# google/neural-light-transport

Hardware: AMD Instinct MI355X
Metric: rendered Mtexels/s at 1024^2 UV (full Model.call forward: U-Net + UV->camera warp); at N > 1: N collective-free replicas of this forward (weak scaling).  The data-parallel TRAIN step with the RCCL gradient all-reduce (BASELINE config 4) is `train_step`: value = Mtexels/s over all ranks, speedup_vs_o (higher is better)
Workload: dtype f32 via 3xbf16 split, 9 exact products, fp32 accumulate (the LDS-tiled encoder convs: fp32 operands as three bf16 terms on v_mfma_f32_16x16x32_bf16, every term product exact in fp32); f32 storage everywhere, every other launch native f32; 1 GPU; BASELINE config 3: dragon_specular relight+view-synth, depth0 16/depth 256, 4 frames/GPU, 1024^2 UV, k=4 obs maps, 512^2 camera warp; frames_per_gpu=4, uv=1024, k=4, cam=512, conv_algo=auto, plan=fused ends, launch=eager, two HIP streams, distinct_batches_rotated=3, launch_tape_replays=0, parallelism=dp1 (frames sharded, no forward collective), world=1, dist_world_size=1, device=cuda:0

## Files before the change

neural-light-transport_amd/csrc/conv_tile3.hip:

```cpp
#include "nlt_common.h"
#include "pack_common.h"

namespace {

typedef __attribute__((ext_vector_type(8))) __bf16 bf16x8;
typedef unsigned short u16;
typedef unsigned int u32x4 __attribute__((ext_vector_type(4)));

constexpr int TH = 8, TW = 16;
constexpr int QS2 = 272, ODD2 = 132;
constexpr int PL = 160;

template <int MODE> struct T3;
template <> struct T3<NLT_CONV_K2S1> { static constexpr int PAIRS = 2, B_UNITS = 153 * 2, B_SLOTS = 6 * PL; };
template <> struct T3<NLT_CONV_K2S2> { static constexpr int PAIRS = 1, B_UNITS = 256 * 2, B_SLOTS = 6 * QS2; };

struct Tile3P {
  const float* src; const u16* packed; const float* bias;
  float* out; float* mean_out;
  int ld, cin, frames, kobs, h, w;
  int oh, ow, cout, ldo, ldm;
  int tiles_y, tiles_x, ncc;
  int act; float alpha;
};

__device__ __forceinline__ int xcd_tile3(int b, int nblocks) {
  return (nblocks & 7) ? b : (b & 7) * (nblocks >> 3) + (b >> 3);
}

__device__ __forceinline__ unsigned cvt_pk_bf16(float a, float b) {
  typedef float f32x2_ __attribute__((ext_vector_type(2)));
  typedef __bf16 bf16x2_ __attribute__((ext_vector_type(2)));
  return __builtin_bit_cast(unsigned, __builtin_convertvector((f32x2_){a, b}, bf16x2_));
}

__device__ __forceinline__ void split2(float a, float b, unsigned& hi, unsigned& mid, unsigned& lo) {
  hi = cvt_pk_bf16(a, b);
  const float ra = a - __uint_as_float(hi << 16), rb = b - __uint_as_float(hi & 0xffff0000u);
  mid = cvt_pk_bf16(ra, rb);
  const float sa = ra - __uint_as_float(mid << 16), sb = rb - __uint_as_float(mid & 0xffff0000u);
  lo = cvt_pk_bf16(sa, sb);
}

__host__ __device__ inline u16 bf16_rne_bits(float f) {
  union { float f; unsigned u; } x; x.f = f;
  x.u += 0x7fffu + ((x.u >> 16) & 1u);
  return (u16)(x.u >> 16);
}
__host__ __device__ inline float bf16_bits_float(u16 b) {
  union { float f; unsigned u; } x; x.u = (unsigned)b << 16;
  return x.f;
}

__global__ void pack_tile3_kernel(const float* __restrict__ wk, int cin, int cout, int tnt, long total, u16* __restrict__ wp) {
  const long idx = (long)blockIdx.x * blockDim.x + threadIdx.x;
  if (idx >= total) return;
  const int e = idx & 7, lane = (idx >> 3) & 63;
  long r = idx >> 9;
  const int term = r % 3; r /= 3;
  const int ct = r % tnt; r /= tnt;
  const int pair = r & 1; r >>= 1;
  const int ncc = cin >> 4;
  const int cc = r % ncc;
  const int g = r / ncc;
  const int kk = lane >> 4, i = lane & 15;
  const int t = pair * 2 + (kk >> 1);
  const int c = cc * 16 + (kk & 1) * 8 + e;
  const int o = (g * tnt + ct) * 16 + i;
  const float v = wk[((long)t * cin + c) * cout + o];
  const u16 hi = bf16_rne_bits(v);
  const float r1 = v - bf16_bits_float(hi);
  const u16 mid = bf16_rne_bits(r1);
  const float r2 = r1 - bf16_bits_float(mid);
  wp[idx] = term == 0 ? hi : (term == 1 ? mid : bf16_rne_bits(r2));
}

template <int MODE, int TNT, int NPROD, int KO>
__global__ __launch_bounds__(256, 2) void conv_tile3_kernel(Tile3P p) {
  using TT = T3<MODE>;
  constexpr int WN = TNT == 4 ? 2 : 1, WM = 4 / WN, RT = TH / WM, CT = 2;
  constexpr int A_SLOTS = TT::PAIRS * TNT * 3 * 64;
  constexpr int NA = (A_SLOTS + 255) / 256, NB = (TT::B_UNITS + 255) / 256;
  __shared__ u32x4 lds[2 * A_SLOTS + 2 * TT::B_SLOTS];

  const int tid = threadIdx.x, lane = tid & 63, wave = tid >> 6;
  const int kk = lane >> 4, j = lane & 15;
  const int wn = wave % WN, wm = wave / WN;
  int tile = xcd_tile3(blockIdx.x, gridDim.x);
  const int tx0 = (tile % p.tiles_x) * TW; tile /= p.tiles_x;
  const int ty0 = (tile % p.tiles_y) * TH;
  const int f = tile / p.tiles_y;
  const int g = blockIdx.y;
  const int spf = (MODE == NLT_CONV_K2S1 ? 1 : 2) * p.ncc;
  const int groups = p.kobs / KO;
  const int total = spf * p.kobs;
  const long in_frame = (long)p.h * p.w;

  int b_lds[NB], b_hf[NB]; long b_tex[NB]; bool b_ok[NB], b_st[NB];
#pragma unroll
  for (int i = 0; i < NB; ++i) {
    const int u = tid + 256 * i;
    const int hf = (u >> 3) & 1, tx = (u >> 4) * 8 + (u & 7);
    b_hf[i] = hf;
    if (MODE == NLT_CONV_K2S1) {
      const int hy = tx / 17, hx = tx % 17;
      const int gy = ty0 + hy, gx = tx0 + hx;
      b_st[i] = tx < 153;
      b_ok[i] = b_st[i] && gy < p.h && gx < p.w;
      b_tex[i] = (long)gy * p.w + gx;
      b_lds[i] = hf * PL + tx;
    } else {
      const int y = tx >> 5, xx = tx & 31;
      const int gy = 2 * (ty0 + y), gx = 2 * tx0 + xx;
      b_st[i] = tx < 256;
      b_ok[i] = b_st[i] && (ty0 + y) < p.oh && gx < p.w;
      b_tex[i] = (long)gy * p.w + gx;
      b_lds[i] = hf * QS2 + (xx & 1) * ODD2 + y * 16 + (xx >> 1);
    }
  }
  constexpr int BPL = MODE == NLT_CONV_K2S1 ? PL : QS2;

  u32x4 ra[NA];
  f32x4 rb[NB][2];
  auto load_a = [&](int s) {
    const int cc = MODE == NLT_CONV_K2S1 ? s : (s >> 1);
    const int a = MODE == NLT_CONV_K2S1 ? 0 : (s & 1);
    const u32x4* ap = reinterpret_cast<const u32x4*>(p.packed) + (((long)g * p.ncc + cc) * 2 + a) * (TNT * 3 * 64);
#pragma unroll
    for (int n = 0; n < NA; ++n) ra[n] = ap[(A_SLOTS % 256 == 0 || tid + 256 * n < A_SLOTS) ? tid + 256 * n : tid];
  };
  auto load_b = [&](int s, int frame) {
    const int cc = MODE == NLT_CONV_K2S1 ? s : (s >> 1);
    const int a = MODE == NLT_CONV_K2S1 ? 0 : (s & 1);
    const float* sp = p.src + ((long)(f * p.kobs + frame) * in_frame + (long)a * p.w) * p.ld + cc * 16;
#pragma unroll
    for (int n = 0; n < NB; ++n) {
      const float* q8 = sp + (b_ok[n] ? b_tex[n] : 0) * p.ld + 8 * b_hf[n];
      const f32x4 v0 = *reinterpret_cast<const f32x4*>(q8), v1 = *reinterpret_cast<const f32x4*>(q8 + 4);
      const f32x4 z = {0.f, 0.f, 0.f, 0.f};
      rb[n][0] = b_ok[n] ? v0 : z;
      rb[n][1] = b_ok[n] ? v1 : z;
    }
  };
  auto store_a = [&](int buf) {
    u32x4* base = lds + buf * A_SLOTS;
#pragma unroll
    for (int n = 0; n < NA; ++n)
      if (A_SLOTS % 256 == 0 || tid + 256 * n < A_SLOTS) base[tid + 256 * n] = ra[n];
  };
  auto store_b = [&](int buf) {
    u32x4* base = lds + 2 * A_SLOTS + buf * TT::B_SLOTS;
#pragma unroll
    for (int n = 0; n < NB; ++n) {
      if (!b_st[n]) continue;
      unsigned hi[4], mid[4], lo[4];
      split2(rb[n][0][0], rb[n][0][1], hi[0], mid[0], lo[0]);
      split2(rb[n][0][2], rb[n][0][3], hi[1], mid[1], lo[1]);
      split2(rb[n][1][0], rb[n][1][1], hi[2], mid[2], lo[2]);
      split2(rb[n][1][2], rb[n][1][3], hi[3], mid[3], lo[3]);
      u32x4* bb = base + b_lds[n];
      bb[0] = (u32x4){hi[0], hi[1], hi[2], hi[3]};
      bb[2 * BPL] = (u32x4){mid[0], mid[1], mid[2], mid[3]};
      bb[4 * BPL] = (u32x4){lo[0], lo[1], lo[2], lo[3]};
    }
  };

  f32x4 acc[KO][RT][CT], mean[RT][CT];
#pragma unroll
  for (int rt = 0; rt < RT; ++rt)
#pragma unroll
    for (int ct = 0; ct < CT; ++ct) {
      mean[rt][ct] = (f32x4){0.f, 0.f, 0.f, 0.f};
#pragma unroll
      for (int io = 0; io < KO; ++io) acc[io][rt][ct] = mean[rt][ct];
    }

  load_a(0);
  load_b(0, 0);
  store_a(0);
  store_b(0);
  __syncthreads();
  int q = 0;
  for (int gi = 0; gi < groups; ++gi) {
    for (int s = 0; s < spf; ++s) {
      const int sa = (gi * spf + s) & 1;
#pragma unroll
      for (int io = 0; io < KO; ++io, ++q) {
        const bool more = q + 1 < total;
        const bool new_slab = io + 1 == KO;
        int ns = s, ngi = gi;
        if (new_slab) { if (++ns == spf) { ns = 0; ++ngi; } }
        if (more) {
          if (new_slab) load_a(ns);
          load_b(ns, ngi * KO + (new_slab ? 0 : io + 1));
        }
        const u32x4* A = lds + sa * A_SLOTS;
        const u32x4* B = lds + 2 * A_SLOTS + (q & 1) * TT::B_SLOTS;
#pragma unroll
        for (int pl = 0; pl < TT::PAIRS; ++pl) {
          bf16x8 bt[3][RT], at[3][CT];
#pragma unroll
          for (int rt = 0; rt < RT; ++rt) {
            const int y = wm * RT + rt;
            const int slot = MODE == NLT_CONV_K2S1 ? (kk & 1) * PL + (y + pl) * 17 + j + (kk >> 1)
                                                   : (kk & 1) * QS2 + (kk >> 1) * ODD2 + y * 16 + j;
#pragma unroll
            for (int t = 0; t < 3; ++t) bt[t][rt] = __builtin_bit_cast(bf16x8, B[t * 2 * BPL + slot]);
          }
#pragma unroll
          for (int ct = 0; ct < CT; ++ct)
#pragma unroll
            for (int t = 0; t < 3; ++t)
              at[t][ct] = __builtin_bit_cast(bf16x8, A[((pl * TNT + wn * CT + ct) * 3 + t) * 64 + lane]);
          constexpr int ORDER9[9][2] = {{2, 2}, {2, 1}, {1, 2}, {2, 0}, {0, 2}, {1, 1}, {1, 0}, {0, 1}, {0, 0}};
#pragma unroll
          for (int pi = 9 - NPROD; pi < 9; ++pi)
#pragma unroll
            for (int rt = 0; rt < RT; ++rt)
#pragma unroll
              for (int ct = 0; ct < CT; ++ct)
                acc[io][rt][ct] = __builtin_amdgcn_mfma_f32_16x16x32_bf16(at[ORDER9[pi][0]][ct], bt[ORDER9[pi][1]][rt], acc[io][rt][ct], 0, 0, 0);
        }
        if (s == spf - 1 && io == KO - 1) {
#pragma unroll
          for (int e = 0; e < KO; ++e) {
            const int i = gi * KO + e;
#pragma unroll
            for (int ct = 0; ct < CT; ++ct) {
              const int oc = (g * TNT + wn * CT + ct) * 16 + 4 * kk;
              const f32x4 bv = *reinterpret_cast<const f32x4*>(p.bias + oc);
#pragma unroll
              for (int rt = 0; rt < RT; ++rt) {
                const int gy = ty0 + wm * RT + rt, gx = tx0 + j;
                f32x4 v = acc[e][rt][ct] + bv;
                if (p.act) {
#pragma unroll
                  for (int c4 = 0; c4 < 4; ++c4) v[c4] = v[c4] > 0.f ? v[c4] : p.alpha * v[c4];
                }
                acc[e][rt][ct] = (f32x4){0.f, 0.f, 0.f, 0.f};
                mean[rt][ct] += v;
                if (gy < p.oh && gx < p.ow) {
                  const long ot = ((long)(f * p.kobs + i) * p.oh + gy) * p.ow + gx;
                  if (p.out) *reinterpret_cast<f32x4*>(p.out + ot * p.ldo + oc) = v;
                  if (p.mean_out && i == p.kobs - 1) {
                    const long mt = ((long)f * p.oh + gy) * p.ow + gx;
                    *reinterpret_cast<f32x4*>(p.mean_out + mt * p.ldm + oc) = mean[rt][ct] * (1.f / (float)p.kobs);
                  }
                }
              }
            }
          }
        }
        if (more) {
          if (new_slab) store_a(sa ^ 1);
          store_b((q + 1) & 1);
        }
        __syncthreads();
      }
    }
  }
}

extern __shared__ u32x4 tile3r_lds[];

template <int MODE, int TNT, int NPROD, int KO, int NWV>
__global__ __launch_bounds__(64 * NWV, 2) void conv_tile3r_kernel(Tile3P p, int ngroups) {
  using TT = T3<MODE>;
  constexpr int NT = 64 * NWV;
  constexpr int WN = TNT == 4 ? 2 : 1, WM = NWV / WN, RT = TH / WM, CT = 2;
  constexpr int A_SLOTS = TT::PAIRS * TNT * 3 * 64;
  constexpr int NB = (TT::B_UNITS + NT - 1) / NT;
  constexpr int BPL = MODE == NLT_CONV_K2S1 ? PL : QS2;
  const int a_group = p.ncc * 2 * TNT * 3 * 64;
  u32x4* const lds_b = tile3r_lds + a_group;

  const int tid = threadIdx.x, lane = tid & 63, wave = tid >> 6;
  const int kk = lane >> 4, j = lane & 15;
  const int wn = wave % WN, wm = wave / WN;
  const int spf = (MODE == NLT_CONV_K2S1 ? 1 : 2) * p.ncc;
  const int groups = p.kobs / KO;
  const long in_frame = (long)p.h * p.w;
  const int tiles = p.frames * p.tiles_y * p.tiles_x;
  const long items = (long)tiles * ngroups;
  const int rank = xcd_tile3(blockIdx.x, gridDim.x);
  int it = (int)(rank * items / gridDim.x);
  const int it_end = (int)((rank + 1) * items / gridDim.x);
  if (it >= it_end) return;

  int b_lds[NB], b_hf[NB]; long b_tex[NB]; bool b_ok[NB], b_st[NB];
#pragma unroll
  for (int i = 0; i < NB; ++i) {
    const int u = tid + NT * i;
    const int hf = (u >> 3) & 1, tx = (u >> 4) * 8 + (u & 7);
    b_hf[i] = hf;
    if (MODE == NLT_CONV_K2S1) {
      b_st[i] = tx < 153;
      b_lds[i] = hf * PL + tx;
    } else {
      const int y = tx >> 5, xx = tx & 31;
      b_st[i] = tx < 256;
      b_lds[i] = hf * QS2 + (xx & 1) * ODD2 + y * 16 + (xx >> 1);
    }
  }
  int ng = 0, nf = 0, nty0 = 0, ntx0 = 0;
  auto geom = [&](int item) {
    ng = item / tiles;
    int t = item - ng * tiles;
    ntx0 = (t % p.tiles_x) * TW; t /= p.tiles_x;
    nty0 = (t % p.tiles_y) * TH;
    nf = t / p.tiles_y;
#pragma unroll
    for (int i = 0; i < NB; ++i) {
      const int u = tid + NT * i;
      const int tx = (u >> 4) * 8 + (u & 7);
      if (MODE == NLT_CONV_K2S1) {
        const int gy = nty0 + tx / 17, gx = ntx0 + tx % 17;
        b_ok[i] = b_st[i] && gy < p.h && gx < p.w;
        b_tex[i] = (long)gy * p.w + gx;
      } else {
        const int y = tx >> 5, xx = tx & 31;
        const int gy = 2 * (nty0 + y), gx = 2 * ntx0 + xx;
        b_ok[i] = b_st[i] && (nty0 + y) < p.oh && gx < p.w;
        b_tex[i] = (long)gy * p.w + gx;
      }
    }
  };

  f32x4 rb[NB][2];
  auto load_b = [&](int s, int frame) {
    const int cc = MODE == NLT_CONV_K2S1 ? s : (s >> 1);
    const int a = MODE == NLT_CONV_K2S1 ? 0 : (s & 1);
    const float* sp = p.src + ((long)(nf * p.kobs + frame) * in_frame + (long)a * p.w) * p.ld + cc * 16;
#pragma unroll
    for (int n = 0; n < NB; ++n) {
      const float* q8 = sp + (b_ok[n] ? b_tex[n] : 0) * p.ld + 8 * b_hf[n];
      const f32x4 v0 = *reinterpret_cast<const f32x4*>(q8), v1 = *reinterpret_cast<const f32x4*>(q8 + 4);
      const f32x4 z = {0.f, 0.f, 0.f, 0.f};
      rb[n][0] = b_ok[n] ? v0 : z;
      rb[n][1] = b_ok[n] ? v1 : z;
    }
  };
  auto store_b = [&](int buf) {
    u32x4* base = lds_b + buf * TT::B_SLOTS;
#pragma unroll
    for (int n = 0; n < NB; ++n) {
      if (!b_st[n]) continue;
      unsigned hi[4], mid[4], lo[4];
      split2(rb[n][0][0], rb[n][0][1], hi[0], mid[0], lo[0]);
      split2(rb[n][0][2], rb[n][0][3], hi[1], mid[1], lo[1]);
      split2(rb[n][1][0], rb[n][1][1], hi[2], mid[2], lo[2]);
      split2(rb[n][1][2], rb[n][1][3], hi[3], mid[3], lo[3]);
      u32x4* bb = base + b_lds[n];
      bb[0] = (u32x4){hi[0], hi[1], hi[2], hi[3]};
      bb[2 * BPL] = (u32x4){mid[0], mid[1], mid[2], mid[3]};
      bb[4 * BPL] = (u32x4){lo[0], lo[1], lo[2], lo[3]};
    }
  };
  auto copy_a = [&](int grp) {
    const u32x4* ap = reinterpret_cast<const u32x4*>(p.packed) + (long)grp * a_group;
    for (int i = tid; i < a_group; i += NT) tile3r_lds[i] = ap[i];
  };

  f32x4 acc[KO][RT][CT], mean[RT][CT];
#pragma unroll
  for (int rt = 0; rt < RT; ++rt)
#pragma unroll
    for (int ct = 0; ct < CT; ++ct) {
      mean[rt][ct] = (f32x4){0.f, 0.f, 0.f, 0.f};
#pragma unroll
      for (int io = 0; io < KO; ++io) acc[io][rt][ct] = mean[rt][ct];
    }

  geom(it);
  load_b(0, 0);
  copy_a(ng);
  store_b(0);
  __syncthreads();
  int q = 0;
  for (; it < it_end; ++it) {
    const int g = ng, f = nf, ty0 = nty0, tx0 = ntx0;
    const bool last_item = it + 1 == it_end;
    for (int gi = 0; gi < groups; ++gi) {
      for (int s = 0; s < spf; ++s) {
#pragma unroll
        for (int io = 0; io < KO; ++io, ++q) {
          const bool new_slab = io + 1 == KO;
          int ns = s, ngi = gi;
          if (new_slab) { if (++ns == spf) { ns = 0; ++ngi; } }
          const bool item_end = ngi == groups;
          if (item_end) {
            ngi = 0;
            if (!last_item) geom(it + 1);
          }
          load_b(ns, ngi * KO + (new_slab ? 0 : io + 1));
          const u32x4* A = tile3r_lds + s * A_SLOTS;
          const u32x4* B = lds_b + (q & 1) * TT::B_SLOTS;
#pragma unroll
          for (int pl = 0; pl < TT::PAIRS; ++pl) {
            bf16x8 bt[3][RT], at[3][CT];
#pragma unroll
            for (int rt = 0; rt < RT; ++rt) {
              const int y = wm * RT + rt;
              const int slot = MODE == NLT_CONV_K2S1 ? (kk & 1) * PL + (y + pl) * 17 + j + (kk >> 1)
                                                     : (kk & 1) * QS2 + (kk >> 1) * ODD2 + y * 16 + j;
#pragma unroll
              for (int t = 0; t < 3; ++t) bt[t][rt] = __builtin_bit_cast(bf16x8, B[t * 2 * BPL + slot]);
            }
#pragma unroll
            for (int ct = 0; ct < CT; ++ct)
#pragma unroll
              for (int t = 0; t < 3; ++t)
                at[t][ct] = __builtin_bit_cast(bf16x8, A[((pl * TNT + wn * CT + ct) * 3 + t) * 64 + lane]);
            constexpr int ORDER9[9][2] = {{2, 2}, {2, 1}, {1, 2}, {2, 0}, {0, 2}, {1, 1}, {1, 0}, {0, 1}, {0, 0}};
#pragma unroll
            for (int pi = 9 - NPROD; pi < 9; ++pi)
#pragma unroll
              for (int rt = 0; rt < RT; ++rt)
#pragma unroll
                for (int ct = 0; ct < CT; ++ct)
                  acc[io][rt][ct] = __builtin_amdgcn_mfma_f32_16x16x32_bf16(at[ORDER9[pi][0]][ct], bt[ORDER9[pi][1]][rt], acc[io][rt][ct], 0, 0, 0);
          }
          if (s == spf - 1 && io == KO - 1) {
#pragma unroll
            for (int e = 0; e < KO; ++e) {
              const int i = gi * KO + e;
#pragma unroll
              for (int ct = 0; ct < CT; ++ct) {
                const int oc = (g * TNT + wn * CT + ct) * 16 + 4 * kk;
                const f32x4 bv = *reinterpret_cast<const f32x4*>(p.bias + oc);
#pragma unroll
                for (int rt = 0; rt < RT; ++rt) {
                  const int gy = ty0 + wm * RT + rt, gx = tx0 + j;
                  f32x4 v = acc[e][rt][ct] + bv;
                  if (p.act) {
#pragma unroll
                    for (int c4 = 0; c4 < 4; ++c4) v[c4] = v[c4] > 0.f ? v[c4] : p.alpha * v[c4];
                  }
                  acc[e][rt][ct] = (f32x4){0.f, 0.f, 0.f, 0.f};
                  mean[rt][ct] += v;
                  if (gy < p.oh && gx < p.ow) {
                    const long ot = ((long)(f * p.kobs + i) * p.oh + gy) * p.ow + gx;
                    if (p.out) *reinterpret_cast<f32x4*>(p.out + ot * p.ldo + oc) = v;
                    if (p.mean_out && i == p.kobs - 1) {
                      const long mt = ((long)f * p.oh + gy) * p.ow + gx;
                      *reinterpret_cast<f32x4*>(p.mean_out + mt * p.ldm + oc) = mean[rt][ct] * (1.f / (float)p.kobs);
                    }
                  }
                  if (i == p.kobs - 1) mean[rt][ct] = (f32x4){0.f, 0.f, 0.f, 0.f};
                }
              }
            }
          }
          if (!(item_end && last_item)) store_b((q + 1) & 1);
          __syncthreads();
        }
      }
    }
    if (!last_item && ng != g) {
      copy_a(ng);
      __syncthreads();
    }
  }
}

constexpr size_t TILE3R_LDS_CU = 160 * 1024;

int tile3r_cus() {
  static const int n = [] {
    int dev = 0, v = 0;
    if (hipGetDevice(&dev) != hipSuccess) return 0;
    if (hipDeviceGetAttribute(&v, hipDeviceAttributeMultiprocessorCount, dev) != hipSuccess) return 0;
    return v;
  }();
  return n;
}

int tile3r_allow_lds(const void* kernel, size_t lds, size_t (&done)[8]) {
  int dev = 0;
  if (lds <= 64 * 1024) return NLT_OK;
  if (hipGetDevice(&dev) != hipSuccess) return NLT_ERR_LAUNCH;
  if (dev >= 0 && dev < 8 && done[dev] >= lds) return NLT_OK;
  if (hipFuncSetAttribute(kernel, hipFuncAttributeMaxDynamicSharedMemorySize, (int)lds) != hipSuccess) return NLT_ERR_LAUNCH;
  if (dev >= 0 && dev < 8) done[dev] = lds;
  return NLT_OK;
}

template <int MODE, int TNT, int NPROD, int KO, int NWV>
int launch3r_k(const Tile3P& p, size_t lds, int nwg, hipStream_t s) {
  auto* k = conv_tile3r_kernel<MODE, TNT, NPROD, KO, NWV>;
  static size_t done[8] = {};
  if (tile3r_allow_lds(reinterpret_cast<const void*>(k), lds, done) != NLT_OK) return NLT_ERR_LAUNCH;
  hipLaunchKernelGGL(k, dim3((unsigned)nwg), dim3(64 * NWV), lds, s, p, p.cout / (16 * TNT));
  NLT_CHECK_LAUNCH();
  return NLT_OK;
}

template <int RT, int NPROD>
__global__ __launch_bounds__(512, 2) void conv_tile3w_kernel(Tile3P p, int ngroups, int tiles_y) {
  constexpr int TNT = 2, CT = 2, NWV = 8;
  constexpr int ROWS = RT + 1, UNITS = ROWS * 17 * 2, NB = (UNITS + 63) / 64;
  constexpr int PLW = (ROWS * 17 + 15) / 16 * 16;
  constexpr int A_SLOTS = 2 * TNT * 3 * 64;
  const int a_group = p.ncc * A_SLOTS;
  const int tid = threadIdx.x, lane = tid & 63, wave = tid >> 6;
  const int kk = lane >> 4, j = lane & 15;
  u32x4* const B = tile3r_lds + a_group + wave * (6 * PLW);
  const long in_frame = (long)p.h * p.w;
  const int tiles = p.frames * tiles_y * p.tiles_x;
  const long items = (long)tiles * ngroups;
  const int rank = xcd_tile3(blockIdx.x, gridDim.x);
  const int it0 = (int)(rank * items / gridDim.x), it1 = (int)((rank + 1) * items / gridDim.x);

  int b_lds[NB], b_hf[NB], b_tx[NB]; long b_tex[NB]; bool b_ok[NB], b_st[NB];
#pragma unroll
  for (int i = 0; i < NB; ++i) {
    const int u = lane + 64 * i;
    b_hf[i] = (u >> 3) & 1;
    b_tx[i] = (u >> 4) * 8 + (u & 7);
    b_st[i] = b_tx[i] < ROWS * 17;
    b_lds[i] = b_hf[i] * PLW + b_tx[i];
  }
  int nf = 0, nty0 = 0, ntx0 = 0;
  auto geom = [&](int t) {
    ntx0 = (t % p.tiles_x) * TW; t /= p.tiles_x;
    nty0 = (t % tiles_y) * RT;
    nf = t / tiles_y;
#pragma unroll
    for (int i = 0; i < NB; ++i) {
      const int gy = nty0 + b_tx[i] / 17, gx = ntx0 + b_tx[i] % 17;
      b_ok[i] = b_st[i] && gy < p.h && gx < p.w;
      b_tex[i] = (long)gy * p.w + gx;
    }
  };
  f32x4 rb[NB][2];
  auto load_b = [&](int cc, int frame) {
    const float* sp = p.src + (long)(nf * p.kobs + frame) * in_frame * p.ld + cc * 16;
#pragma unroll
    for (int n = 0; n < NB; ++n) {
      const float* q8 = sp + (b_ok[n] ? b_tex[n] : 0) * p.ld + 8 * b_hf[n];
      const f32x4 v0 = *reinterpret_cast<const f32x4*>(q8), v1 = *reinterpret_cast<const f32x4*>(q8 + 4);
      const f32x4 z = {0.f, 0.f, 0.f, 0.f};
      rb[n][0] = b_ok[n] ? v0 : z;
      rb[n][1] = b_ok[n] ? v1 : z;
    }
  };
  auto store_b = [&]() {
#pragma unroll
    for (int n = 0; n < NB; ++n) {
      if (!b_st[n]) continue;
      unsigned hi[4], mid[4], lo[4];
      split2(rb[n][0][0], rb[n][0][1], hi[0], mid[0], lo[0]);
      split2(rb[n][0][2], rb[n][0][3], hi[1], mid[1], lo[1]);
      split2(rb[n][1][0], rb[n][1][1], hi[2], mid[2], lo[2]);
      split2(rb[n][1][2], rb[n][1][3], hi[3], mid[3], lo[3]);
      u32x4* bb = B + b_lds[n];
      bb[0] = (u32x4){hi[0], hi[1], hi[2], hi[3]};
      bb[2 * PLW] = (u32x4){mid[0], mid[1], mid[2], mid[3]};
      bb[4 * PLW] = (u32x4){lo[0], lo[1], lo[2], lo[3]};
    }
  };
  auto wave_sync = [&]() {
    __builtin_amdgcn_fence(__ATOMIC_RELEASE, "wavefront");
    __builtin_amdgcn_wave_barrier();
    __builtin_amdgcn_fence(__ATOMIC_ACQUIRE, "wavefront");
  };

  int seg = it0;
  while (seg < it1) {
    const int g = seg / tiles;
    const int seg_end = min(it1, (g + 1) * tiles);
    {
      const u32x4* ap = reinterpret_cast<const u32x4*>(p.packed) + (long)g * a_group;
      for (int i = tid; i < a_group; i += 64 * NWV) tile3r_lds[i] = ap[i];
    }
    __syncthreads();
    int it = seg + wave;
    if (it < seg_end) {
      f32x4 acc[RT][CT], mean[RT][CT];
#pragma unroll
      for (int rt = 0; rt < RT; ++rt)
#pragma unroll
        for (int ct = 0; ct < CT; ++ct) acc[rt][ct] = mean[rt][ct] = (f32x4){0.f, 0.f, 0.f, 0.f};
      geom(it - g * tiles);
      load_b(0, 0);
      store_b();
      wave_sync();
      for (; it < seg_end; it += NWV) {
        const int f = nf, ty0 = nty0, tx0 = ntx0;
        const bool last_item = it + NWV >= seg_end;
        for (int i = 0; i < p.kobs; ++i) {
          for (int s = 0; s < p.ncc; ++s) {
            int ns = s + 1, ni = i;
            if (ns == p.ncc) { ns = 0; ++ni; }
            const bool item_end = ni == p.kobs;
            if (item_end) {
              ni = 0;
              if (!last_item) geom(it + NWV - g * tiles);
            }
            load_b(ns, ni);
            bf16x8 bt[3][ROWS];
#pragma unroll
            for (int r = 0; r < ROWS; ++r)
#pragma unroll
              for (int t = 0; t < 3; ++t)
                bt[t][r] = __builtin_bit_cast(bf16x8, B[t * 2 * PLW + (kk & 1) * PLW + r * 17 + j + (kk >> 1)]);
            wave_sync();
            const u32x4* A = tile3r_lds + s * A_SLOTS;
#pragma unroll
            for (int pl = 0; pl < 2; ++pl) {
              bf16x8 at[3][CT];
#pragma unroll
              for (int ct = 0; ct < CT; ++ct)
#pragma unroll
                for (int t = 0; t < 3; ++t) at[t][ct] = __builtin_bit_cast(bf16x8, A[((pl * TNT + ct) * 3 + t) * 64 + lane]);
              constexpr int ORDER9[9][2] = {{2, 2}, {2, 1}, {1, 2}, {2, 0}, {0, 2}, {1, 1}, {1, 0}, {0, 1}, {0, 0}};
#pragma unroll
              for (int pi = 9 - NPROD; pi < 9; ++pi)
#pragma unroll
                for (int rt = 0; rt < RT; ++rt)
#pragma unroll
                  for (int ct = 0; ct < CT; ++ct)
                    acc[rt][ct] = __builtin_amdgcn_mfma_f32_16x16x32_bf16(at[ORDER9[pi][0]][ct], bt[ORDER9[pi][1]][rt + pl], acc[rt][ct], 0, 0, 0);
            }
            if (!(item_end && last_item)) store_b();
            wave_sync();
            if (s == p.ncc - 1) {
#pragma unroll
              for (int ct = 0; ct < CT; ++ct) {
                const int oc = (g * TNT + ct) * 16 + 4 * kk;
                const f32x4 bv = *reinterpret_cast<const f32x4*>(p.bias + oc);
#pragma unroll
                for (int rt = 0; rt < RT; ++rt) {
                  const int gy = ty0 + rt, gx = tx0 + j;
                  f32x4 v = acc[rt][ct] + bv;
                  if (p.act) {
#pragma unroll
                    for (int c4 = 0; c4 < 4; ++c4) v[c4] = v[c4] > 0.f ? v[c4] : p.alpha * v[c4];
                  }
                  acc[rt][ct] = (f32x4){0.f, 0.f, 0.f, 0.f};
                  mean[rt][ct] += v;
                  if (gy < p.oh && gx < p.ow) {
                    const long ot = ((long)(f * p.kobs + i) * p.oh + gy) * p.ow + gx;
                    if (p.out) *reinterpret_cast<f32x4*>(p.out + ot * p.ldo + oc) = v;
                    if (p.mean_out && i == p.kobs - 1) {
                      const long mt = ((long)f * p.oh + gy) * p.ow + gx;
                      *reinterpret_cast<f32x4*>(p.mean_out + mt * p.ldm + oc) = mean[rt][ct] * (1.f / (float)p.kobs);
                    }
                  }
                  if (i == p.kobs - 1) mean[rt][ct] = (f32x4){0.f, 0.f, 0.f, 0.f};
                }
              }
            }
          }
        }
      }
    }
    seg = seg_end;
    if (seg < it1) __syncthreads();
  }
}

template <int RT>
int launch3w(const Tile3P& p, int nprod, int max_wg, hipStream_t s) {
  constexpr int PLW = ((RT + 1) * 17 + 15) / 16 * 16;
  const size_t lds = (size_t)p.cin * 2 * 384 + 8 * 6 * PLW * sizeof(u32x4);
  if (lds > TILE3R_LDS_CU) return NLT_ERR_UNSUPPORTED;
  const int cus = tile3r_cus();
  if (cus <= 0) return NLT_ERR_LAUNCH;
  const int tiles_y = (p.oh + RT - 1) / RT;
  const long items = (long)p.frames * tiles_y * p.tiles_x * (p.cout / 32);
  long nwg = cus;
  if (max_wg > 0 && nwg > max_wg) nwg = max_wg;
  if (nwg > items) nwg = items;
  auto* k = nprod == 9 ? conv_tile3w_kernel<RT, 9> : conv_tile3w_kernel<RT, 6>;
  static size_t done[2][8] = {};
  if (tile3r_allow_lds(reinterpret_cast<const void*>(k), lds, done[nprod == 9]) != NLT_OK) return NLT_ERR_LAUNCH;
  hipLaunchKernelGGL(k, dim3((unsigned)nwg), dim3(512), lds, s, p, p.cout / 32, tiles_y);
  NLT_CHECK_LAUNCH();
  return NLT_OK;
}

template <int MODE, int TNT, int KO>
int launch3r(const Tile3P& p, int nprod, int max_wg, hipStream_t s) {
  if (nprod != 6 && nprod != 9) return NLT_ERR_UNSUPPORTED;
  if (MODE == NLT_CONV_K2S1 && TNT == 2) {
    int st = launch3w<4>(p, nprod, max_wg, s);
    if (st == NLT_ERR_UNSUPPORTED) st = launch3w<2>(p, nprod, max_wg, s);
    if (st != NLT_ERR_UNSUPPORTED) return st;
  }
  const size_t lds = (size_t)p.cin * TNT * 384 + 2 * T3<MODE>::B_SLOTS * sizeof(u32x4);
  if (lds > TILE3R_LDS_CU) return NLT_ERR_UNSUPPORTED;
  const bool wide = 2 * lds > TILE3R_LDS_CU;
  const int cus = tile3r_cus();
  if (cus <= 0) return NLT_ERR_LAUNCH;
  const long items = (long)p.frames * p.tiles_y * p.tiles_x * (p.cout / (16 * TNT));
  long nwg = (long)cus * (wide ? 1 : 2);
  if (max_wg > 0 && nwg > max_wg) nwg = max_wg;
  if (nwg > items) nwg = items;
  if (items >= (1l << 31)) return NLT_ERR_UNSUPPORTED;
  if (wide) return nprod == 9 ? launch3r_k<MODE, TNT, 9, KO, 8>(p, lds, (int)nwg, s) : launch3r_k<MODE, TNT, 6, KO, 8>(p, lds, (int)nwg, s);
  return nprod == 9 ? launch3r_k<MODE, TNT, 9, KO, 4>(p, lds, (int)nwg, s) : launch3r_k<MODE, TNT, 6, KO, 4>(p, lds, (int)nwg, s);
}

template <int MODE, int TNT, int KO>
int launch3k(const Tile3P& p, int nprod, hipStream_t s, int resident_wg) {
  if (resident_wg >= 0) return launch3r<MODE, TNT, KO>(p, nprod, resident_wg, s);
  const long tiles = (long)p.frames * p.tiles_y * p.tiles_x;
  const dim3 grid((unsigned)tiles, (unsigned)(p.cout / (16 * TNT)));
  if (nprod == 9) hipLaunchKernelGGL((conv_tile3_kernel<MODE, TNT, 9, KO>), grid, dim3(256), 0, s, p);
  else if (nprod == 6) hipLaunchKernelGGL((conv_tile3_kernel<MODE, TNT, 6, KO>), grid, dim3(256), 0, s, p);
  else if (KO > 1) return NLT_ERR_UNSUPPORTED;
  else if (nprod == 3) hipLaunchKernelGGL((conv_tile3_kernel<MODE, TNT, 3, 1>), grid, dim3(256), 0, s, p);
  else hipLaunchKernelGGL((conv_tile3_kernel<MODE, TNT, 1, 1>), grid, dim3(256), 0, s, p);
  NLT_CHECK_LAUNCH();
  return NLT_OK;
}

template <int MODE, int TNT>
int launch3(const Tile3P& p, int nprod, hipStream_t s, int resident_wg) {
  static const int want = [] { const char* e = getenv("NLT_TILE3_KO"); return e ? atoi(e) : 0; }();
  const int cap = want > 0 ? want : (TNT == 2 ? 4 : (MODE == NLT_CONV_K2S1 || resident_wg >= 0 ? 1 : 2));
  if (nprod >= 6) {
    if (TNT == 2 && cap >= 4 && p.kobs % 4 == 0) return launch3k<MODE, TNT, (TNT == 2 ? 4 : 1)>(p, nprod, s, resident_wg);
    if (cap >= 2 && p.kobs % 2 == 0) return launch3k<MODE, TNT, 2>(p, nprod, s, resident_wg);
  }
  return launch3k<MODE, TNT, 1>(p, nprod, s, resident_wg);
}

}

extern "C" long nlt_conv_tile3_packed_elems(int mode, int cin, int cout, int tn) {
  if ((mode != NLT_CONV_K2S1 && mode != NLT_CONV_K2S2) || cin <= 0 || cout <= 0) return -1;
  if ((cin & 15) || (tn != 32 && tn != 64) || cout % tn) return -1;
  return (long)12 * cin * cout;
}

extern "C" int nlt_pack_conv_tile3_weights(int mode, const float* w_keras, int cin, int cout, int tn, unsigned short* packed,
                                           void* stream) {
  const long total = nlt_conv_tile3_packed_elems(mode, cin, cout, tn);
  if (total <= 0) return NLT_ERR_UNSUPPORTED;
  if (!w_keras || !packed || !nlt_aligned16(packed)) return NLT_ERR_BAD_ARG;
  hipLaunchKernelGGL(pack_tile3_kernel, dim3((unsigned)((total + 255) / 256)), dim3(256), 0, static_cast<hipStream_t>(stream),
                     w_keras, cin, cout, tn / 16, total, packed);
  NLT_CHECK_LAUNCH();
  return NLT_OK;
}

static int tile3_forward(int mode, int nprod, const float* src, int ld, int cin, int frames, int kobs, int h, int w,
                         const unsigned short* packed, const float* bias, int cout, int tn,
                         float* out, int ldo, float* mean_out, int ldm, int act, float alpha, int resident_wg, void* stream) {
  if (!src || !packed || !bias || (!out && !mean_out) || (nprod != 1 && nprod != 3 && nprod != 6 && nprod != 9)) return NLT_ERR_BAD_ARG;
  if (frames <= 0 || kobs <= 0 || h <= 0 || w <= 0 || cin <= 0 || cout <= 0) return NLT_ERR_BAD_ARG;
  if (nlt_conv_tile3_packed_elems(mode, cin, cout, tn) <= 0) return NLT_ERR_UNSUPPORTED;
  if (mode == NLT_CONV_K2S2 && ((h | w) & 1)) return NLT_ERR_UNSUPPORTED;
  if (ld < cin || (ld & 3) || (out && (ldo < cout || (ldo & 3))) || (mean_out && (ldm < cout || (ldm & 3)))) return NLT_ERR_BAD_ARG;
  if (!nlt_aligned16(src) || !nlt_aligned16(packed) || !nlt_aligned16(bias) || (out && !nlt_aligned16(out)) ||
      (mean_out && !nlt_aligned16(mean_out))) return NLT_ERR_BAD_ARG;
  if ((long long)frames * kobs * h * w * (long long)(ld > ldo ? ld : ldo) >= (1ll << 31)) return NLT_ERR_UNSUPPORTED;
  Tile3P p;
  p.src = src; p.packed = packed; p.bias = bias; p.out = out; p.mean_out = mean_out;
  p.ld = ld; p.cin = cin; p.frames = frames; p.kobs = kobs; p.h = h; p.w = w;
  p.oh = mode == NLT_CONV_K2S2 ? h / 2 : h; p.ow = mode == NLT_CONV_K2S2 ? w / 2 : w;
  p.cout = cout; p.ldo = ldo; p.ldm = ldm; p.ncc = cin / 16; p.act = act; p.alpha = alpha;
  p.tiles_y = (p.oh + TH - 1) / TH; p.tiles_x = (p.ow + TW - 1) / TW;
  hipStream_t s = static_cast<hipStream_t>(stream);
  if (mode == NLT_CONV_K2S1)
    return tn == 64 ? launch3<NLT_CONV_K2S1, 4>(p, nprod, s, resident_wg) : launch3<NLT_CONV_K2S1, 2>(p, nprod, s, resident_wg);
  return tn == 64 ? launch3<NLT_CONV_K2S2, 4>(p, nprod, s, resident_wg) : launch3<NLT_CONV_K2S2, 2>(p, nprod, s, resident_wg);
}

extern "C" int nlt_conv_tile3_forward(int mode, int nprod, const float* src, int ld, int cin, int frames, int kobs, int h, int w,
                                      const unsigned short* packed, const float* bias, int cout, int tn,
                                      float* out, int ldo, float* mean_out, int ldm, int act, float alpha, void* stream) {
  return tile3_forward(mode, nprod, src, ld, cin, frames, kobs, h, w, packed, bias, cout, tn, out, ldo, mean_out, ldm, act, alpha,
                       -1, stream);
}

extern "C" int nlt_conv_tile3r_forward(int mode, int nprod, const float* src, int ld, int cin, int frames, int kobs, int h, int w,
                                       const unsigned short* packed, const float* bias, int cout, int tn,
                                       float* out, int ldo, float* mean_out, int ldm, int act, float alpha, int max_workgroups,
                                       void* stream) {
  if (max_workgroups < 0) return NLT_ERR_BAD_ARG;
  return tile3_forward(mode, nprod, src, ld, cin, frames, kobs, h, w, packed, bias, cout, tn, out, ldo, mean_out, ldm, act, alpha,
                       max_workgroups, stream);
}
```

Baseline: 3622 Mtexels/s.

## Add direct-register resident kernel for stride-2 encoder convs, bypassing LDS B staging

Adds a persistent conv_tile3d kernel for the 2x2 stride-2 convs. Each wave owns an output tile, loads its input texels straight into registers and splits them into three bf16 terms there, and double-buffers the next slab's loads and splits between the MFMA products. Weights stay resident in LDS per output-channel group. This drops the shared B-tile staging, its barriers and its LDS footprint. The old resident kernel is specialised to stride-1 only, and a heuristic (tile3d_pays, overridable by env) falls back to the non-resident path for small channel counts. The trade-off is that neighbouring waves no longer share input via LDS, so global load traffic per wave rises, and register pressure rises too.

Measured after the change: 3664 Mtexels/s (median of 3 runs). 1.01x the previous value.

```diff
diff --git a/neural-light-transport_amd/csrc/conv_tile3.hip b/neural-light-transport_amd/csrc/conv_tile3.hip
--- a/neural-light-transport_amd/csrc/conv_tile3.hip
+++ b/neural-light-transport_amd/csrc/conv_tile3.hip
@@ -1,3 +1,5 @@
+#include <type_traits>
+
 #include "nlt_common.h"
 #include "pack_common.h"
 
@@ -263,21 +265,21 @@
 
 extern __shared__ u32x4 tile3r_lds[];
 
-template <int MODE, int TNT, int NPROD, int KO, int NWV>
+template <int TNT, int NPROD, int KO, int NWV>
 __global__ __launch_bounds__(64 * NWV, 2) void conv_tile3r_kernel(Tile3P p, int ngroups) {
-  using TT = T3<MODE>;
+  using TT = T3<NLT_CONV_K2S1>;
   constexpr int NT = 64 * NWV;
   constexpr int WN = TNT == 4 ? 2 : 1, WM = NWV / WN, RT = TH / WM, CT = 2;
   constexpr int A_SLOTS = TT::PAIRS * TNT * 3 * 64;
   constexpr int NB = (TT::B_UNITS + NT - 1) / NT;
-  constexpr int BPL = MODE == NLT_CONV_K2S1 ? PL : QS2;
+  constexpr int BPL = PL;
   const int a_group = p.ncc * 2 * TNT * 3 * 64;
   u32x4* const lds_b = tile3r_lds + a_group;
 
   const int tid = threadIdx.x, lane = tid & 63, wave = tid >> 6;
   const int kk = lane >> 4, j = lane & 15;
   const int wn = wave % WN, wm = wave / WN;
-  const int spf = (MODE == NLT_CONV_K2S1 ? 1 : 2) * p.ncc;
+  const int spf = p.ncc;
   const int groups = p.kobs / KO;
   const long in_frame = (long)p.h * p.w;
   const int tiles = p.frames * p.tiles_y * p.tiles_x;
@@ -293,14 +295,8 @@
     const int u = tid + NT * i;
     const int hf = (u >> 3) & 1, tx = (u >> 4) * 8 + (u & 7);
     b_hf[i] = hf;
-    if (MODE == NLT_CONV_K2S1) {
-      b_st[i] = tx < 153;
-      b_lds[i] = hf * PL + tx;
-    } else {
-      const int y = tx >> 5, xx = tx & 31;
-      b_st[i] = tx < 256;
-      b_lds[i] = hf * QS2 + (xx & 1) * ODD2 + y * 16 + (xx >> 1);
-    }
+    b_st[i] = tx < 153;
+    b_lds[i] = hf * PL + tx;
   }
   int ng = 0, nf = 0, nty0 = 0, ntx0 = 0;
   auto geom = [&](int item) {
@@ -313,24 +309,15 @@
     for (int i = 0; i < NB; ++i) {
       const int u = tid + NT * i;
       const int tx = (u >> 4) * 8 + (u & 7);
-      if (MODE == NLT_CONV_K2S1) {
-        const int gy = nty0 + tx / 17, gx = ntx0 + tx % 17;
-        b_ok[i] = b_st[i] && gy < p.h && gx < p.w;
-        b_tex[i] = (long)gy * p.w + gx;
-      } else {
-        const int y = tx >> 5, xx = tx & 31;
-        const int gy = 2 * (nty0 + y), gx = 2 * ntx0 + xx;
-        b_ok[i] = b_st[i] && (nty0 + y) < p.oh && gx < p.w;
-        b_tex[i] = (long)gy * p.w + gx;
-      }
+      const int gy = nty0 + tx / 17, gx = ntx0 + tx % 17;
+      b_ok[i] = b_st[i] && gy < p.h && gx < p.w;
+      b_tex[i] = (long)gy * p.w + gx;
     }
   };
 
   f32x4 rb[NB][2];
   auto load_b = [&](int s, int frame) {
-    const int cc = MODE == NLT_CONV_K2S1 ? s : (s >> 1);
-    const int a = MODE == NLT_CONV_K2S1 ? 0 : (s & 1);
-    const float* sp = p.src + ((long)(nf * p.kobs + frame) * in_frame + (long)a * p.w) * p.ld + cc * 16;
+    const float* sp = p.src + (long)(nf * p.kobs + frame) * in_frame * p.ld + s * 16;
 #pragma unroll
     for (int n = 0; n < NB; ++n) {
       const float* q8 = sp + (b_ok[n] ? b_tex[n] : 0) * p.ld + 8 * b_hf[n];
@@ -401,8 +388,7 @@
 #pragma unroll
             for (int rt = 0; rt < RT; ++rt) {
               const int y = wm * RT + rt;
-              const int slot = MODE == NLT_CONV_K2S1 ? (kk & 1) * PL + (y + pl) * 17 + j + (kk >> 1)
-                                                     : (kk & 1) * QS2 + (kk >> 1) * ODD2 + y * 16 + j;
+              const int slot = (kk & 1) * PL + (y + pl) * 17 + j + (kk >> 1);
 #pragma unroll
               for (int t = 0; t < 3; ++t) bt[t][rt] = __builtin_bit_cast(bf16x8, B[t * 2 * BPL + slot]);
             }
@@ -485,9 +471,9 @@
   return NLT_OK;
 }
 
-template <int MODE, int TNT, int NPROD, int KO, int NWV>
+template <int TNT, int NPROD, int KO, int NWV>
 int launch3r_k(const Tile3P& p, size_t lds, int nwg, hipStream_t s) {
-  auto* k = conv_tile3r_kernel<MODE, TNT, NPROD, KO, NWV>;
+  auto* k = conv_tile3r_kernel<TNT, NPROD, KO, NWV>;
   static size_t done[8] = {};
   if (tile3r_allow_lds(reinterpret_cast<const void*>(k), lds, done) != NLT_OK) return NLT_ERR_LAUNCH;
   hipLaunchKernelGGL(k, dim3((unsigned)nwg), dim3(64 * NWV), lds, s, p, p.cout / (16 * TNT));
@@ -680,15 +666,203 @@
   return NLT_OK;
 }
 
-template <int MODE, int TNT, int KO>
+template <int RT, int TNT, int NPROD, int NWV>
+__global__ __launch_bounds__(64 * NWV, NWV == 4 ? 2 : 1) void conv_tile3d_kernel(Tile3P p, int ngroups, int tiles_y) {
+  constexpr int CT = TNT, A_STAGE = TNT * 3 * 64;
+  const int a_group = 2 * p.ncc * A_STAGE;
+  const int tid = threadIdx.x, lane = tid & 63, wave = __builtin_amdgcn_readfirstlane(tid >> 6);
+  const int kk = lane >> 4, j = lane & 15;
+  const long in_frame = (long)p.h * p.w;
+  const int tiles = p.frames * tiles_y * p.tiles_x;
+  const long items = (long)tiles * ngroups;
+  const int rank = xcd_tile3(blockIdx.x, gridDim.x);
+  const int it0 = (int)(rank * items / gridDim.x), it1 = (int)((rank + 1) * items / gridDim.x);
+  const int lane_off = (kk >> 1) * p.ld + 8 * (kk & 1);
+
+  int l_it = 0, l_i = 0, l_cc = 0, l_f = 0, l_ty0 = 0, l_tx0 = 0;
+  int tex[RT]; bool ok[RT];
+  auto geom = [&](int t) {
+    l_tx0 = (t % p.tiles_x) * TW; t /= p.tiles_x;
+    l_ty0 = (t % tiles_y) * RT;
+    l_f = t / tiles_y;
+    const int x = l_tx0 + j;
+#pragma unroll
+    for (int rt = 0; rt < RT; ++rt) {
+      const int y = l_ty0 + rt;
+      ok[rt] = y < p.oh && x < p.ow;
+      tex[rt] = (2 * min(y, p.oh - 1) * p.w + 2 * min(x, p.ow - 1)) * p.ld + lane_off;
+    }
+  };
+  f32x4 raw[2][RT][2];
+  u32x4 bt[2][3][RT];
+  auto load = [&](auto ac) {
+    constexpr int a = decltype(ac)::value;
+    const float* sp = p.src + ((long)(l_f * p.kobs + l_i) * in_frame + (long)a * p.w) * p.ld + l_cc * 16;
+#pragma unroll
+    for (int rt = 0; rt < RT; ++rt) {
+      const float* q8 = sp + tex[rt];
+      raw[a][rt][0] = *reinterpret_cast<const f32x4*>(q8);
+      raw[a][rt][1] = *reinterpret_cast<const f32x4*>(q8 + 4);
+    }
+  };
+  auto split_unit = [&](auto ac, int u, const bool (&okv)[RT]) {
+    constexpr int a = decltype(ac)::value;
+    const int rt = u >> 2, q = u & 3;
+    const f32x4 v = raw[a][rt][q >> 1];
+    const float x0 = okv[rt] ? v[(q & 1) * 2] : 0.f, x1 = okv[rt] ? v[(q & 1) * 2 + 1] : 0.f;
+    unsigned hi, mid, lo;
+    split2(x0, x1, hi, mid, lo);
+    bt[a][0][rt][q] = hi; bt[a][1][rt][q] = mid; bt[a][2][rt][q] = lo;
+  };
+
+  int seg = it0;
+  while (seg < it1) {
+    const int g = seg / tiles;
+    const int seg_end = min(it1, (g + 1) * tiles);
+    {
+      const u32x4* ap = reinterpret_cast<const u32x4*>(p.packed) + (long)g * a_group;
+      for (int i = tid; i < a_group; i += 64 * NWV) tile3r_lds[i] = ap[i];
+    }
+    __syncthreads();
+    const int it = seg + wave;
+    if (it < seg_end) {
+      f32x4 acc[RT][CT], mean[RT][CT], bv[CT];
+#pragma unroll
+      for (int ct = 0; ct < CT; ++ct) bv[ct] = *reinterpret_cast<const f32x4*>(p.bias + (g * TNT + ct) * 16 + 4 * kk);
+#pragma unroll
+      for (int rt = 0; rt < RT; ++rt)
+#pragma unroll
+        for (int ct = 0; ct < CT; ++ct) acc[rt][ct] = mean[rt][ct] = (f32x4){0.f, 0.f, 0.f, 0.f};
+      const int ndouble = (seg_end - it + NWV - 1) / NWV * p.kobs * p.ncc;
+      l_it = it; l_i = 0; l_cc = 0;
+      geom(it - g * tiles);
+      load(std::integral_constant<int, 0>{});
+      load(std::integral_constant<int, 1>{});
+#pragma unroll
+      for (int u = 0; u < 4 * RT; ++u) split_unit(std::integral_constant<int, 0>{}, u, ok);
+      for (int d = 0; d < ndouble; ++d) {
+        const int f = l_f, ty0 = l_ty0, tx0 = l_tx0, i = l_i, cc = l_cc;
+        bool okc[RT];
+#pragma unroll
+        for (int rt = 0; rt < RT; ++rt) okc[rt] = ok[rt];
+        {
+          const bool slab_end = l_cc + 1 == p.ncc, obs_end = slab_end && l_i + 1 == p.kobs;
+          const bool next_item = obs_end && l_it + NWV < seg_end;
+          l_cc = slab_end ? 0 : l_cc + 1;
+          l_i = obs_end ? 0 : (slab_end ? l_i + 1 : l_i);
+          l_it = next_item ? l_it + NWV : l_it;
+          geom(l_it - g * tiles);
+        }
+        auto stage = [&](auto ac, auto nc, const bool (&okn)[RT]) {
+          constexpr int a = decltype(ac)::value;
+          load(ac);
+          __builtin_amdgcn_sched_barrier(0);
+          const u32x4* A = tile3r_lds + (2 * cc + a) * A_STAGE;
+          bf16x8 at[3][CT];
+#pragma unroll
+          for (int ct = 0; ct < CT; ++ct)
+#pragma unroll
+            for (int t = 0; t < 3; ++t) at[t][ct] = __builtin_bit_cast(bf16x8, A[(ct * 3 + t) * 64 + lane]);
+          constexpr int ORDER9[9][2] = {{2, 2}, {2, 1}, {1, 2}, {2, 0}, {0, 2}, {1, 1}, {1, 0}, {0, 1}, {0, 0}};
+#pragma unroll
+          for (int pi = 9 - NPROD; pi < 9; ++pi) {
+#pragma unroll
+            for (int rt = 0; rt < RT; ++rt)
+#pragma unroll
+              for (int ct = 0; ct < CT; ++ct)
+                acc[rt][ct] = __builtin_amdgcn_mfma_f32_16x16x32_bf16(at[ORDER9[pi][0]][ct], __builtin_bit_cast(bf16x8, bt[a][ORDER9[pi][1]][rt]),
+                                                                      acc[rt][ct], 0, 0, 0);
+            constexpr int P0 = 9 - NPROD;
+#pragma unroll
+            for (int u = (pi - P0) * 4 * RT / NPROD; u < (pi - P0 + 1) * 4 * RT / NPROD; ++u) split_unit(nc, u, okn);
+            __builtin_amdgcn_sched_barrier(0);
+          }
+          constexpr int n = decltype(nc)::value;
+#pragma unroll
+          for (int t = 0; t < 3; ++t)
+#pragma unroll
+            for (int rt = 0; rt < RT; ++rt) asm volatile("" : "+v"(bt[n][t][rt]));
+        };
+        stage(std::integral_constant<int, 0>{}, std::integral_constant<int, 1>{}, okc);
+        stage(std::integral_constant<int, 1>{}, std::integral_constant<int, 0>{}, ok);
+        if (cc == p.ncc - 1) {
+#pragma unroll
+          for (int ct = 0; ct < CT; ++ct) {
+            const int oc = (g * TNT + ct) * 16 + 4 * kk;
+#pragma unroll
+            for (int rt = 0; rt < RT; ++rt) {
+              const int gy = ty0 + rt, gx = tx0 + j;
+              f32x4 v = acc[rt][ct] + bv[ct];
+              if (p.act) {
+#pragma unroll
+                for (int c4 = 0; c4 < 4; ++c4) v[c4] = v[c4] > 0.f ? v[c4] : p.alpha * v[c4];
+              }
+              acc[rt][ct] = (f32x4){0.f, 0.f, 0.f, 0.f};
+              mean[rt][ct] += v;
+              if (gy < p.oh && gx < p.ow) {
+                const long ot = ((long)(f * p.kobs + i) * p.oh + gy) * p.ow + gx;
+                if (p.out) *reinterpret_cast<f32x4*>(p.out + ot * p.ldo + oc) = v;
+                if (p.mean_out && i == p.kobs - 1) {
+                  const long mt = ((long)f * p.oh + gy) * p.ow + gx;
+                  *reinterpret_cast<f32x4*>(p.mean_out + mt * p.ldm + oc) = mean[rt][ct] * (1.f / (float)p.kobs);
+                }
+              }
+              if (i == p.kobs - 1) mean[rt][ct] = (f32x4){0.f, 0.f, 0.f, 0.f};
+            }
+          }
+        }
+      }
+    }
+    seg = seg_end;
+    if (seg < it1) __syncthreads();
+  }
+}
+
+template <int RT, int TNT, int NWV>
+int launch3d_k(const Tile3P& p, int nprod, int max_wg, hipStream_t s) {
+  const size_t lds = (size_t)p.cin * TNT * 384;
+  const int cus = tile3r_cus();
+  if (cus <= 0) return NLT_ERR_LAUNCH;
+  const int tiles_y = (p.oh + RT - 1) / RT;
+  const long items = (long)p.frames * tiles_y * p.tiles_x * (p.cout / (16 * TNT));
+  if (items >= (1l << 31)) return NLT_ERR_UNSUPPORTED;
+  long nwg = NWV == 4 && 2 * lds <= TILE3R_LDS_CU ? 2 * cus : cus;
+  if (max_wg > 0 && nwg > max_wg) nwg = max_wg;
+  if (nwg > items) nwg = items;
+  auto* k = nprod == 9 ? conv_tile3d_kernel<RT, TNT, 9, NWV> : conv_tile3d_kernel<RT, TNT, 6, NWV>;
+  static size_t done[2][8] = {};
+  if (tile3r_allow_lds(reinterpret_cast<const void*>(k), lds, done[nprod == 9]) != NLT_OK) return NLT_ERR_LAUNCH;
+  hipLaunchKernelGGL(k, dim3((unsigned)nwg), dim3(64 * NWV), lds, s, p, p.cout / (16 * TNT), tiles_y);
+  NLT_CHECK_LAUNCH();
+  return NLT_OK;
+}
+
+int tile3d_want() { const char* e = getenv("NLT_TILE3D"); return e ? atoi(e) : 0; }
+
+bool tile3d_pays(int cin, int cout) { return tile3d_want() != 0 || 2l * cin * cout >= 32l * (4 * cin + cout); }
+
+template <int TNT>
+int launch3d(const Tile3P& p, int nprod, int max_wg, hipStream_t s) {
+  if (nprod != 6 && nprod != 9) return NLT_ERR_UNSUPPORTED;
+  if ((size_t)p.cin * TNT * 384 > TILE3R_LDS_CU) return NLT_ERR_UNSUPPORTED;
+  const int want = tile3d_want();
+  if (want == 204) return launch3d_k<2, TNT, 4>(p, nprod, max_wg, s);
+  if constexpr (TNT == 2) {
+    if (want == 212) return launch3d_k<2, TNT, 12>(p, nprod, max_wg, s);
+    if (want == 408) return launch3d_k<4, TNT, 8>(p, nprod, max_wg, s);
+  }
+  return launch3d_k<2, TNT, 8>(p, nprod, max_wg, s);
+}
+
+template <int TNT, int KO>
 int launch3r(const Tile3P& p, int nprod, int max_wg, hipStream_t s) {
   if (nprod != 6 && nprod != 9) return NLT_ERR_UNSUPPORTED;
-  if (MODE == NLT_CONV_K2S1 && TNT == 2) {
+  if (TNT == 2) {
     int st = launch3w<4>(p, nprod, max_wg, s);
     if (st == NLT_ERR_UNSUPPORTED) st = launch3w<2>(p, nprod, max_wg, s);
     if (st != NLT_ERR_UNSUPPORTED) return st;
   }
-  const size_t lds = (size_t)p.cin * TNT * 384 + 2 * T3<MODE>::B_SLOTS * sizeof(u32x4);
+  const size_t lds = (size_t)p.cin * TNT * 384 + 2 * T3<NLT_CONV_K2S1>::B_SLOTS * sizeof(u32x4);
   if (lds > TILE3R_LDS_CU) return NLT_ERR_UNSUPPORTED;
   const bool wide = 2 * lds > TILE3R_LDS_CU;
   const int cus = tile3r_cus();
@@ -698,13 +872,16 @@
   if (max_wg > 0 && nwg > max_wg) nwg = max_wg;
   if (nwg > items) nwg = items;
   if (items >= (1l << 31)) return NLT_ERR_UNSUPPORTED;
-  if (wide) return nprod == 9 ? launch3r_k<MODE, TNT, 9, KO, 8>(p, lds, (int)nwg, s) : launch3r_k<MODE, TNT, 6, KO, 8>(p, lds, (int)nwg, s);
-  return nprod == 9 ? launch3r_k<MODE, TNT, 9, KO, 4>(p, lds, (int)nwg, s) : launch3r_k<MODE, TNT, 6, KO, 4>(p, lds, (int)nwg, s);
+  if (wide) return nprod == 9 ? launch3r_k<TNT, 9, KO, 8>(p, lds, (int)nwg, s) : launch3r_k<TNT, 6, KO, 8>(p, lds, (int)nwg, s);
+  return nprod == 9 ? launch3r_k<TNT, 9, KO, 4>(p, lds, (int)nwg, s) : launch3r_k<TNT, 6, KO, 4>(p, lds, (int)nwg, s);
 }
 
 template <int MODE, int TNT, int KO>
 int launch3k(const Tile3P& p, int nprod, hipStream_t s, int resident_wg) {
-  if (resident_wg >= 0) return launch3r<MODE, TNT, KO>(p, nprod, resident_wg, s);
+  if (resident_wg >= 0) {
+    if constexpr (MODE == NLT_CONV_K2S2) return launch3d<TNT>(p, nprod, resident_wg, s);
+    else return launch3r<TNT, KO>(p, nprod, resident_wg, s);
+  }
   const long tiles = (long)p.frames * p.tiles_y * p.tiles_x;
   const dim3 grid((unsigned)tiles, (unsigned)(p.cout / (16 * TNT)));
   if (nprod == 9) hipLaunchKernelGGL((conv_tile3_kernel<MODE, TNT, 9, KO>), grid, dim3(256), 0, s, p);
@@ -764,6 +941,11 @@
   p.cout = cout; p.ldo = ldo; p.ldm = ldm; p.ncc = cin / 16; p.act = act; p.alpha = alpha;
   p.tiles_y = (p.oh + TH - 1) / TH; p.tiles_x = (p.ow + TW - 1) / TW;
   hipStream_t s = static_cast<hipStream_t>(stream);
+  if (mode == NLT_CONV_K2S2 && resident_wg >= 0) {
+    if (nprod != 6 && nprod != 9) return NLT_ERR_UNSUPPORTED;
+    if ((size_t)cin * (tn / 16) * 384 > TILE3R_LDS_CU) return NLT_ERR_UNSUPPORTED;
+    if (!tile3d_pays(cin, cout)) resident_wg = -1;
+  }
   if (mode == NLT_CONV_K2S1)
     return tn == 64 ? launch3<NLT_CONV_K2S1, 4>(p, nprod, s, resident_wg) : launch3<NLT_CONV_K2S1, 2>(p, nprod, s, resident_wg);
   return tn == 64 ? launch3<NLT_CONV_K2S2, 4>(p, nprod, s, resident_wg) : launch3<NLT_CONV_K2S2, 2>(p, nprod, s, resident_wg);
```
